# MattAgostini/ECE1782-Smith-Waterman-CUDA

Hardware: AMD Instinct MI355X
Metric: GCUPS (DP cell updates/s) query-vs-SwissProt, 1/2/4/8 MI355X; bit-exact scores (higher is better)
Workload: dtype fp16

## Files before the change

ece1782-smith-waterman-cuda_amd/csrc/sw_capi.cpp:

```cpp
#include <algorithm>
#include <cmath>
#include <atomic>
#include <cstdio>
#include <cstdlib>
#include <cstring>
#include <memory>
#include <new>
#include <numeric>
#include <string>
#include <thread>
#include <unordered_map>
#include <vector>

#include "sw_host.h"
#include "sw_plan.h"

using swk::DevPtr;
using swk::Event;
using swk::HostPtr;
using swk::Stream;

namespace {

thread_local std::string g_err;
// ... 1085 lines not shown
    }
    if ((p.multi_inter || p.multi_intra) && (rc = ensure_bnd(db, p.affine, p.intra_x2))) return rc;
    if (p.intra_x2 && !db->lay.d_lrescue.get()) {
        HIPCHECK(swk::dev_alloc(db->lay.d_lrescue, 2 * lstride * sizeof(int32_t)));
        HIPCHECK(hipMemsetAsync(db->lay.d_lrescue.get(), 0xff, 2 * lstride * sizeof(int32_t), h->stream.get()));
        db->lay.device_bytes += 2 * lstride * sizeof(int32_t);
    }
    if (db->list_epoch != g_fault_epoch.load()) {
        if ((rc = join_tails(h))) return rc;
        hipStream_t const s = h->stream.get();
        if (int32_t* l = db->lay.d_rescue.get()) HIPCHECK(hipMemsetAsync(l, 0xff, 2 * rstride * sizeof(int32_t), s));
        if (int32_t* l = db->lay.d_lrescue.get()) HIPCHECK(hipMemsetAsync(l, 0xff, 2 * lstride * sizeof(int32_t), s));
        db->list_epoch = g_fault_epoch.load();
    }
    c.par = h->parity;
    h->parity ^= 1;
    if (h->tail_pending[c.par]) {
        HIPCHECK(hipStreamWaitEvent(h->stream.get(), h->tail_done[c.par].get(), 0));
        h->tail_pending[c.par] = false;
    }
    if (p.drain && (rc = join_tails(h))) return rc;
    if (db->lay.d_rescue.get()) {
        c.listA = db->lay.d_rescue.get() + c.par * rstride;
        c.listB = c.listA + db->nblocks + 1;
        c.maxA = c.listA + 2 * (db->nblocks + 1);
        c.headA = c.maxA + 2;
        if (p.lpt && h->opts.lpt_persist != 0) c.lpt_next = c.maxA + 1;
    }
    if (db->lay.d_lrescue.get()) {
        c.list1 = db->lay.d_lrescue.get() + c.par * lstride;
        c.list2 = c.list1 + db->nlong + 1;
        c.head1 = c.list2 + db->nlong + 1;
    }
    c.deferred = !p.drain && defer && (!(p.multi_inter || p.multi_intra) || ensure_rbnd(db, p.affine, p.intra_x2));
    return SW_OK;
}

int scan_profiles(Scan& c, const QuerySrc& src, const int8_t* mat) {
    const swplan::ScanPlan& p = c.plan;
    const bool d = p.drain;
    int32_t* const cA = (p.rescue && c.db->nblocks) ? c.listA : nullptr;
    int32_t* const c1 = p.intra_x2 ? c.list1 : nullptr;
    int32_t* const reset[10] = {cA, (cA && p.f16) ? c.listB : nullptr, (cA && p.f16) ? c.maxA : nullptr, c1,
                                c1 ? c.list2 : nullptr, d ? c.headA : nullptr, d ? c.headA + 1 : nullptr,
                                d ? c.head1 : nullptr, d ? c.head1 + 1 : nullptr, c.lpt_next};
    const int rc = build_profiles(c.h, src, mat, c.sc.go, p.affine,
                                  std::max({p.qpad_inter, p.qpad_rescue, p.qpad_coop, p.qpad_list, p.qpad_intra2}),
                                  p.shape.x2s || p.intra_x2, p.ri, p.qpad_intra, reset, &c.P);
    c.h->evpool[c.h->nscans - 1].merged = p.lpt;
    return rc;
}

int inter_args(Scan& c) {
    sw_db* db = c.db;
    const swplan::ScanPlan& p = c.plan;
    const int go = c.sc.go, ge = c.sc.ge;
    swk::InterArgs& a = c.a;
    a.residues = db->lay.d_res.get();
    a.blk_off = db->lay.d_blk_off.get();
    a.blk_groups = db->lay.d_blk_groups.get();
    a.blk_cols = db->lay.d_blk_cols.get();
    a.lane_ids = db->lay.d_lane_ids.get();
    a.nblocks = static_cast<int32_t>(db->nblocks);
    a.prof = c.P.dev + (p.shape.x2s ? c.P.off16 : c.P.off8);
    a.prof_stride = c.P.stride;
    a.qpad = p.qpad_inter;
    a.gap_open = go;
    a.gap_extend = ge;
    a.bnd_h = db->lay.d_bnd_h.get();
    a.bnd_f = db->lay.d_bnd_f.get();
    a.scores = c.scores;
    if (c.h->opts.trace_file[0]) {
        if (!db->lay.h_trace.get()) {
            db->lay.trace_entries = static_cast<size_t>(2 * db->nblocks + db->nlong + 8);
            HIPCHECK(swk::host_alloc(db->lay.h_trace, 32 * db->lay.trace_entries, hipHostMallocMapped));
            std::memset(db->lay.h_trace.get(), 0, 32 * db->lay.trace_entries);
        }
        HIPCHECK(hipHostGetDevicePointer(reinterpret_cast<void**>(&a.trace), db->lay.h_trace.get(), 0));
    }
    if (p.rescue) {
        a.rescue_count = c.listA;
        a.rescue_list = c.listA + 1;
        if (p.f16) a.rescue_max = c.maxA;
        const int zero = -kF16Span + 2 * ge;
        a.sat_limit = kF16Span - zero - 2 * std::max(c.sc.max_s, 1) - 26 * ge;
        for (int j = 0; j < 32; ++j) a.f16_step[j] = f16_pair(j * ge + zero);
        a.f16_gog = f16_pair(go - ge);
        a.f16_zero = f16_pair(zero);
        a.f16_diff[0] = f16_pair(4 * ge);
        a.f16_diff[1] = f16_pair(8 * ge);
        a.f16_diff[2] = f16_pair(16 * ge);
    }
    a.re_last = p.re_last;
    if (p.lpt) {
        a.blk_first = p.npair;
        a.blk_quad = p.nquad;
        a.blk_tri = p.ntri ? 1 : 0;
        a.blk_tail = static_cast<int32_t>(db->nblocks) - p.ntail;
    } else if (p.npair) {
        a.blk_base = p.nr;
        a.blk_first = std::max(p.npair, p.nr);
    } else {
        a.blk_first = p.ncoop;
    }
    return SW_OK;
}

void intra_args(Scan& c) {
    const sw_db* db = c.db;
    swk::IntraArgs& ia = c.ia;
    ia.residues = db->lay.d_lres.get();
    ia.subj_off = db->lay.d_loff.get();
    ia.subj_len = db->lay.d_llen.get();
    ia.subj_id = db->lay.d_lid.get();
    ia.nsubj = static_cast<int32_t>(db->nlong);
    ia.prof = c.P.dev + c.P.intra_off;
    ia.qpad = c.plan.qpad_intra;
    ia.gap_open = c.sc.go;
    ia.gap_extend = c.sc.ge;
    ia.bnd_h = db->lay.d_lbnd_h.get();
    ia.bnd_f = db->lay.d_lbnd_f.get();
    ia.scores = c.scores;
}

void intra_x2_args(Scan& c) {
    const swplan::ScanPlan& p = c.plan;
    const int go = c.sc.go, ge = c.sc.ge;
    swk::IntraArgs& x = c.x;
    x = c.ia;
    x.prof = c.P.dev + c.P.off16;
    x.prof_stride = c.P.stride;
    x.bias = p.affine ? 0 : go;
    x.qpad = p.qpad_intra2;
    const int zero = -kF16Span + 2 * ge;
    x.sat_limit = kF16Span - zero - 2 * std::max(c.sc.max_s, 1) - swk::intra_bias_rows(p.ri2) * ge;
    for (int j = 0; j < swk::kIntraSteps; ++j) x.f16_step[j] = f16_pair(j * ge + zero);
    x.f16_zero = f16_pair(zero);
    x.f16_gog = f16_pair(go - ge);
    int32_t* const flagged = p.intra_i16_first ? c.list2 : c.list1;
    x.rescue_count = flagged;
    x.rescue_list = flagged + 1;
}

int scan_args(Scan& c) {
    if (c.db->nlong) {
        intra_args(c);
        if (c.plan.intra_x2) intra_x2_args(c);
    }
    return c.db->nblocks ? inter_args(c) : SW_OK;
}

struct RescueStages {
    swk::InterArgs a16, a32;
    swk::IntraArgs i16, i32;
};
RescueStages rescue_stages(const Scan& c, const swk::IntraArgs& x, const BndRows& r, bool in_launch) {
    const swplan::ScanPlan& p = c.plan;
    auto items = [](int32_t* list) { return list ? list + 1 : nullptr; };
    int32_t* const l32 = p.f16 ? c.listB : c.listA;
    RescueStages s{c.a, c.a, x, c.ia};
    s.a16.bnd_h = s.a32.bnd_h = r.h;
    s.a16.bnd_f = s.a32.bnd_f = r.f;
    s.a16.qpad = p.qpad_list;
    s.a16.re_last = p.affine ? 32 : 48;
    s.a32.re_last = swplan::rescue_rows(p.affine);
    s.a16.rescue_list = items(c.listB);
    s.a16.rescue_count = c.listB;
    s.a16.rescue_max = nullptr;
    s.a32.prof = c.P.dev + c.P.off8;
    s.a32.qpad = p.qpad_rescue;
    s.a32.rescue_list = nullptr;
    s.a32.rescue_count = nullptr;
    s.i16.bnd_h = s.i32.bnd_h = r.lh;
    s.i16.bnd_f = s.i32.bnd_f = r.lf;
// ... 1158 lines not shown
```

ece1782-smith-waterman-cuda_amd/csrc/sw_inter_x2.hip:

```cpp
#include <algorithm>

#include "sw_int32.h"
#include "sw_intra_x2.h"
#include "sw_kernels.h"

namespace swk {

typedef short s2 __attribute__((ext_vector_type(2)));
typedef unsigned short u2 __attribute__((ext_vector_type(2)));

__device__ __forceinline__ s2 as_s2(uint32_t x) { return __builtin_bit_cast(s2, x); }
__device__ __forceinline__ uint32_t as_u32(s2 x) { return __builtin_bit_cast(uint32_t, x); }
__device__ __forceinline__ s2 max2(s2 a, s2 b) { return __builtin_elementwise_max(a, b); }
__device__ __forceinline__ s2 usub2(s2 a, u2 g) {
    return __builtin_bit_cast(s2, __builtin_elementwise_sub_sat(__builtin_bit_cast(u2, a), g));
}

__host__ __device__ constexpr int x2_row_dwords(int R) { return (R / 4) % 2 == 1 ? R : R + 4; }

constexpr int kImgCodes = kPadCode + 1;

template <int R>
struct __attribute__((aligned(16))) X2Lds {
    static constexpr int kImg = kImgCodes * x2_row_dwords(R);
// ... 12 lines not shown
        default: return static_cast<uint32_t>(q.w);
    }
}

template <int SG>
__device__ __forceinline__ void load_codes(uint32_t (&w)[SG / 4], const uint8_t* p, bool valid) {
    if (valid) {
        if constexpr (SG == 16) {
            const int4 v = *reinterpret_cast<const int4*>(p);
            w[0] = v.x; w[1] = v.y; w[2] = v.z; w[3] = v.w;
        } else if constexpr (SG == 8) {
            const int2 v = *reinterpret_cast<const int2*>(p);
            w[0] = v.x; w[1] = v.y;
        } else {
            w[0] = *reinterpret_cast<const uint32_t*>(p);
        }
    } else {
#pragma unroll
        for (int q = 0; q < SG / 4; ++q) w[q] = 0x19191919u;
    }
}

__device__ __forceinline__ uint32_t code_of(const uint32_t* w, int jj) { return (w[jj >> 2] >> (8 * (jj & 3))) & 0xffu; }

template <uint32_t RB>
__device__ __forceinline__ uint32_t code_row(const uint32_t* w, int jj, uint32_t base) {
    static_assert(RB < 256, "row stride must fit a byte");
    return __builtin_amdgcn_udot4(w[jj >> 2], RB << (8 * (jj & 3)), base, false);
}

template <int SG>
__device__ __forceinline__ void load_pairs(uint32_t (&v)[SG], const int32_t* p) {
#pragma unroll
    for (int q = 0; q < SG / 4; ++q) {
        const int4 t = *reinterpret_cast<const int4*>(p + 4 * q);
        v[4 * q] = t.x; v[4 * q + 1] = t.y; v[4 * q + 2] = t.z; v[4 * q + 3] = t.w;
    }
}

template <int SG>
__device__ __forceinline__ void store_pairs(int32_t* p, const uint32_t (&v)[SG]) {
#pragma unroll
    for (int q = 0; q < SG / 4; ++q)
        *reinterpret_cast<int4*>(p + 4 * q) = make_int4(v[4 * q], v[4 * q + 1], v[4 * q + 2], v[4 * q + 3]);
}

__device__ __forceinline__ uint32_t lo_lo(uint32_t a, uint32_t b) { return __builtin_amdgcn_perm(b, a, 0x05040100u); }
__device__ __forceinline__ uint32_t hi_lo(uint32_t a, uint32_t b) { return __builtin_amdgcn_perm(b, a, 0x05040302u); }
__device__ __forceinline__ uint32_t hi_hi(uint32_t a, uint32_t b) { return __builtin_amdgcn_perm(b, a, 0x07060302u); }

template <int SG, bool AFFINE>
__device__ __forceinline__ void load_bnd(uint32_t (&v)[SG], const uint32_t* bnd, uint64_t i) {
    if constexpr (AFFINE) {
        load_pairs<SG>(v, reinterpret_cast<const int32_t*>(bnd) + i);
    } else {
        const uint16_t* p = reinterpret_cast<const uint16_t*>(bnd) + i;
        uint32_t w[SG / 2];
        if constexpr (SG == 8) {
            const int4 t = *reinterpret_cast<const int4*>(p);
            w[0] = t.x; w[1] = t.y; w[2] = t.z; w[3] = t.w;
        } else {
            static_assert(SG == 4, "sub-group width");
            const int2 t = *reinterpret_cast<const int2*>(p);
            w[0] = t.x; w[1] = t.y;
        }
#pragma unroll
        for (int q = 0; q < SG; ++q) v[q] = w[q / 2];
    }
}
template <int SG, bool AFFINE>
__device__ __forceinline__ void store_bnd(uint32_t* bnd, uint64_t i, const uint32_t (&hb)[SG]) {
    if constexpr (AFFINE) {
        store_pairs<SG>(reinterpret_cast<int32_t*>(bnd) + i, hb);
    } else {
        uint16_t* p = reinterpret_cast<uint16_t*>(bnd) + i;
        uint32_t w[SG / 2];
#pragma unroll
        for (int q = 0; q < SG / 2; ++q) w[q] = lo_lo(hb[2 * q], hb[2 * q + 1]);
        if constexpr (SG == 8) *reinterpret_cast<int4*>(p) = make_int4(w[0], w[1], w[2], w[3]);
        else *reinterpret_cast<int2*>(p) = make_int2(w[0], w[1]);
    }
}

__device__ __forceinline__ uint32_t to_f16_bits(uint32_t v16) {
    return static_cast<uint32_t>(__builtin_bit_cast(uint16_t, static_cast<_Float16>(static_cast<int16_t>(v16))));
}

template <int R, bool F16>
__device__ __forceinline__ void stage_x2s(X2Lds<R>& L, const int16_t* __restrict__ prof, int stride, int s0,
                                          int lane, int bias, int bias0, int img, int hi0 = R) {
    constexpr int RD = x2_row_dwords(R);
    constexpr int PER = kImgCodes * (R / 8);
    constexpr uint32_t one = F16 ? 0x3c00u : 1u;
    const int n = img < 0 ? 2 * PER : PER;
    for (int t = lane; t < n; t += kLanes) {
        const int im = img < 0 ? t / PER : img;
        const int u = img < 0 ? t % PER : t;
        const int c = u / (R / 8);
        const int k = u % (R / 8);
        const int16_t* src = prof + static_cast<size_t>(c) * stride + s0 + im * hi0 + 8 * k;
        int4 v;
        if (im && (hi0 & 7)) {
            const int2 v0 = *reinterpret_cast<const int2*>(src), v1 = *reinterpret_cast<const int2*>(src + 4);
            v = make_int4(v0.x, v0.y, v1.x, v1.y);
        } else {
            v = *reinterpret_cast<const int4*>(src);
        }
        const uint32_t w[4] = {static_cast<uint32_t>(v.x), static_cast<uint32_t>(v.y), static_cast<uint32_t>(v.z),
                               static_cast<uint32_t>(v.w)};
        uint32_t o[8];
#pragma unroll
        for (int e = 0; e < 4; ++e) {
            const int s0v = static_cast<int16_t>(w[e] & 0xffffu), s1v = static_cast<int16_t>(w[e] >> 16);
            const int b0 = (F16 && k % 2 == 0 && e == 0) ? bias0 : 0;
            uint32_t a0 = static_cast<uint32_t>(s0v) & 0xffffu, a1 = static_cast<uint32_t>(s1v) & 0xffffu;
            if constexpr (F16) {
                a0 = to_f16_bits(static_cast<uint32_t>(s0v + bias + b0));
                a1 = to_f16_bits(static_cast<uint32_t>(s1v + bias));
            }
            o[2 * e] = im ? (a0 << 16) | one : a0 | (one << 16);
            o[2 * e + 1] = im ? (a1 << 16) | one : a1 | (one << 16);
        }
        int4* d = reinterpret_cast<int4*>((im ? L.hi : L.lo) + c * RD + 8 * k);
        d[0] = make_int4(o[0], o[1], o[2], o[3]);
        d[1] = make_int4(o[4], o[5], o[6], o[7]);
    }
}


typedef int v4i __attribute__((ext_vector_type(4)));
typedef __attribute__((address_space(3))) const v4i lds_int4;

__device__ __forceinline__ uint32_t lds_addr(const void* p) {
    return static_cast<uint32_t>(reinterpret_cast<uintptr_t>(p));
}

template <int N>
__device__ __forceinline__ void read_x2a(int4 (&pl)[N], int4 (&ph)[N], uint32_t& aa, uint32_t& ab, int k,
                                         uint32_t dep) {
    asm volatile("" : "+v"(aa), "+v"(ab) : "v"(dep));
    lds_int4* a = reinterpret_cast<lds_int4*>(static_cast<uintptr_t>(aa)) + N * k;
    lds_int4* b = reinterpret_cast<lds_int4*>(static_cast<uintptr_t>(ab)) + N * k;
#pragma unroll
    for (int q = 0; q < N; ++q) {
        pl[q] = __builtin_bit_cast(int4, a[q]);
        ph[q] = __builtin_bit_cast(int4, b[q]);
    }
}

typedef _Float16 h2 __attribute__((ext_vector_type(2)));

template <bool F16>
struct PkCell;

template <>
struct PkCell<false> {
    using V = s2;
    static __device__ __forceinline__ V from(uint32_t x) { return as_s2(x); }
    static __device__ __forceinline__ uint32_t bits(V x) { return as_u32(x); }
};

template <>
struct PkCell<true> {
    using V = h2;
    static __device__ __forceinline__ V from(uint32_t x) { return __builtin_bit_cast(h2, x); }
    static __device__ __forceinline__ uint32_t bits(V x) { return __builtin_bit_cast(uint32_t, x); }
};

__device__ __forceinline__ h2 max3h(h2 a, h2 b, h2 c) {
    return __builtin_elementwise_maximum(__builtin_elementwise_maximum(a, b), c);
}

template <int R, int SG, bool AFFINE, bool F16, int CR = 16, bool SHORT = true>
__device__ __forceinline__ bool x2s_block(const InterArgs& a, int blk, X2Lds<R>& L, int lane);

template <int R, int SG, bool AFFINE, bool F16, bool LIST, int CR = 16>
__global__ __launch_bounds__(256, 2) void sw_inter_x2s(InterArgs a) {
    static_assert(R % CR == 0 && SG % 4 == 0, "shape");
    __shared__ __attribute__((aligned(16))) X2Lds<R> lds[kWavesPerWG];
    const int wave = __builtin_amdgcn_readfirstlane(threadIdx.x >> 6);
    const int lane = threadIdx.x & 63;
    X2Lds<R>& L = lds[wave];
    if constexpr (LIST) {
        const int n = __builtin_amdgcn_readfirstlane(*a.blk_count);
        for (int i = blockIdx.x * kWavesPerWG + wave; i < n; i += gridDim.x * kWavesPerWG)
            x2s_block<R, SG, AFFINE, F16, CR, false>(a, list_take(a.blk_list, i), L, lane);
        return;
    }
    const int blk = a.blk_first + blockIdx.x * kWavesPerWG + wave;
    if (blk >= a.nblocks) return;
    x2s_block<R, SG, AFFINE, F16, CR>(a, blk, L, lane);
}

constexpr int kRowGroup = 16;
constexpr int kAcc = kRowGroup + 8 - 1;
template <bool F16>
struct Best {
    typename PkCell<F16>::V v;
    __device__ __forceinline__ void init(const InterArgs&) { v = PkCell<F16>::from(0u); }
    __device__ __forceinline__ typename PkCell<F16>::V value(const InterArgs&) const { return v; }
};
template <>
struct Best<true> {
    h2 acc[kAcc];
    __device__ __forceinline__ void init(const InterArgs& a) {
#pragma unroll
        for (int k = 0; k < kAcc; ++k) acc[k] = __builtin_bit_cast(h2, a.f16_zero);
    }
    __device__ __forceinline__ void pin() {
        static_assert(kAcc == 23, "pin list");
        asm volatile("" : "+v"(acc[0]), "+v"(acc[1]), "+v"(acc[2]), "+v"(acc[3]), "+v"(acc[4]), "+v"(acc[5]),
                     "+v"(acc[6]), "+v"(acc[7]));
        asm volatile("" : "+v"(acc[8]), "+v"(acc[9]), "+v"(acc[10]), "+v"(acc[11]), "+v"(acc[12]), "+v"(acc[13]),
                     "+v"(acc[14]), "+v"(acc[15]));
        asm volatile("" : "+v"(acc[16]), "+v"(acc[17]), "+v"(acc[18]), "+v"(acc[19]), "+v"(acc[20]),
                     "+v"(acc[21]), "+v"(acc[22]));
    }
    __device__ __forceinline__ h2 value(const InterArgs& a) const {
        const h2 z = __builtin_bit_cast(h2, a.f16_step[0]);
        h2 b = acc[0];
#pragma unroll
        for (int k = 1; k < kAcc; ++k)
            b = __builtin_elementwise_maximum(b, acc[k] - (__builtin_bit_cast(h2, a.f16_step[k]) - z));
        return b;
    }
};

__device__ __forceinline__ uint64_t trace_now() {
#ifdef SW_TRACE_BLOCKS
    return __builtin_amdgcn_s_memrealtime();
#else
    return 0;
#endif
}
__device__ __forceinline__ void trace_block(const InterArgs& a, int blk, uint64_t t0, int lane, uint32_t kind) {
#ifdef SW_TRACE_BLOCKS
    if (a.trace && lane == 0) {
        const uint64_t t1 = __builtin_amdgcn_s_memrealtime();
        const uint32_t hw = __builtin_amdgcn_s_getreg((4) | (0 << 6) | (31 << 11));
        const uint32_t xcc = __builtin_amdgcn_s_getreg((20) | (0 << 6) | (31 << 11));
        uint64_t* t = a.trace + 4 * static_cast<size_t>(blk);
        t[0] = t0;
        t[1] = t1;
        t[2] = hw;
        t[3] = xcc | (static_cast<uint64_t>(kind) << 32);
    }
#else
    (void)a; (void)blk; (void)t0; (void)lane; (void)kind;
#endif
}

template <bool F16>
__device__ __forceinline__ bool x2s_finish(const InterArgs& a, int blk, int lane, typename PkCell<F16>::V best) {
    int b;
    if constexpr (F16)
        b = static_cast<int>(static_cast<float>(__builtin_elementwise_maximum(best.x, best.y))) -
            static_cast<int>(static_cast<float>(__builtin_bit_cast(h2, a.f16_step[0]).x));
    else
        b = max(static_cast<int>(best.x), static_cast<int>(best.y));
    const int id = a.lane_ids[static_cast<size_t>(blk) * kLanes + lane];
    if (id >= 0) a.scores[id] = b;
    if (a.rescue_list) {
        const bool sat = F16 ? (b >= a.sat_limit) : (b >= kSat16 || b < 0);
        const uint64_t m = __builtin_amdgcn_ballot_w64(sat);
        if (m && lane == 0) {
            list_publish(a.rescue_list, a.rescue_count, blk);
            if (a.rescue_max) atomicMax(a.rescue_max, blk);
        }
        return m != 0;
    }
    return false;
}


constexpr int kRingSlots = 4;

template <int SG>
__device__ __forceinline__ void ring_store(int4* ring, int slot, int lane, const uint32_t (&v)[SG]) {
#pragma unroll
    for (int q = 0; q < SG / 4; ++q)
        ring[(slot * (SG / 4) + q) * kLanes + lane] = make_int4(v[4 * q], v[4 * q + 1], v[4 * q + 2], v[4 * q + 3]);
}

template <int SG>
__device__ __forceinline__ void ring_load(uint32_t (&v)[SG], const int4* ring, int slot, int lane) {
#pragma unroll
    for (int q = 0; q < SG / 4; ++q) {
        const int4 t = ring[(slot * (SG / 4) + q) * kLanes + lane];
        v[4 * q] = static_cast<uint32_t>(t.x);
        v[4 * q + 1] = static_cast<uint32_t>(t.y);
        v[4 * q + 2] = static_cast<uint32_t>(t.z);
        v[4 * q + 3] = static_cast<uint32_t>(t.w);
    }
}

template <bool AFFINE>
constexpr bool pair_flags() { return AFFINE; }
struct PairSync {
    int* prog;
    int me;
    int base;
    int pred;
    int pred_base;
    int succ;
    int S;
};
__device__ __forceinline__ void pair_wait(const int* prog, int wave, int need) {
    while (__hip_atomic_load(prog + wave, __ATOMIC_ACQUIRE, __HIP_MEMORY_SCOPE_WORKGROUP) < need)
        __builtin_amdgcn_s_sleep(1);
}

template <int R, int SG, bool AFFINE, bool F16, bool PAIR, int CR = 16, bool CHAIN = false, int RL = R>
__device__ __forceinline__ void x2s_pass(const InterArgs& a, X2Lds<R>& L, uint32_t ncols, uint64_t base, int lane,
                                         int s0, Best<F16>& best, const int4* ring_in, int4* ring_out,
                                         int* tick, const PairSync* ps = nullptr, int chain_passes = 1) {
    static_assert(!(CHAIN && PAIR), "chained passes: single-wave blocks only");
    constexpr int CQ = CR / 4;
    constexpr int NCH = R / CR;
    constexpr int STEPS = SG * NCH;
    using P = PkCell<F16>;
    using V = typename P::V;
    const int16_t* prof16 = reinterpret_cast<const int16_t*>(a.prof);
    const u2 go2 = {static_cast<unsigned short>(a.gap_open), static_cast<unsigned short>(a.gap_open)};
    const u2 ge2 = {static_cast<unsigned short>(a.gap_extend), static_cast<unsigned short>(a.gap_extend)};
    uint32_t* bnd = reinterpret_cast<uint32_t*>(a.bnd_h);
    static_assert(!F16 || (R % kRowGroup == 0 && SG <= 8), "fp16 row groups");
    h2 gog_h = {}, reb_h = {}, grp_h = {};
    if constexpr (F16) {
        gog_h = __builtin_bit_cast(h2, a.f16_gog);
        static_assert(SG == 4 || SG == 8, "rebase constants");
        reb_h = __builtin_bit_cast(h2, a.f16_diff[SG == 4 ? 0 : 1]);
        grp_h = __builtin_bit_cast(h2, a.f16_diff[2]);
    }
    const bool first = (s0 == 0);
    const bool last = (s0 + 2 * R >= a.qpad);
    const uint32_t npass = CHAIN ? static_cast<uint32_t>(chain_passes) : 1u;
    const bool chain_last = CHAIN && static_cast<int>(npass) * 2 * R >= a.qpad;
    const uint32_t total = npass * ncols;
    const int sbias = F16 ? (AFFINE ? 2 : 1) * a.gap_extend : 0;
    const int gbias0 = F16 ? -kRowGroup * a.gap_extend : 0;
    const uint32_t dtop0 = F16 ? a.f16_step[SG - 2 + kRowGroup] : 0u;
    constexpr bool kSh = RL < R;
    if constexpr (kSh) asm volatile("" : "+v"(lane));
    static_assert(!kSh || (RL == R - 4 && !CHAIN), "rows per strip: R, or R - 4 outside a chain");
    static_assert((R - 4 - 1) % kRowGroup == 11, "the short strip's bottom row: 4 ge under the last row's bias");
    h2 dsh_h = {};
    if constexpr (F16) dsh_h = __builtin_bit_cast(h2, a.f16_diff[0]);
    stage_x2s<R, F16>(L, prof16, a.prof_stride, s0, lane, sbias, gbias0, -1, RL);
    __builtin_amdgcn_fence(__ATOMIC_RELEASE, "workgroup");
    __builtin_amdgcn_wave_barrier();
    __builtin_amdgcn_fence(__ATOMIC_ACQUIRE, "workgroup");

    V H[R];
    V E[AFFINE ? R : 1];
#pragma unroll
    for (int r = 0; r < R; ++r) H[r] = P::from(F16 ? a.f16_step[r % kRowGroup + SG - 1] : 0u);
#pragma unroll
    for (int r = 0; r < (AFFINE ? R : 1); ++r) E[r] = P::from(F16 ? a.f16_zero : 0u);
    uint32_t dtop = dtop0;
    uint32_t dl_h[SG], dl_f[SG];
    uint32_t bin[SG], bin_n[SG];
    uint32_t bz[SG];
    uint32_t rc[SG / 4], rp[SG / 4], rn[SG / 4];
#pragma unroll
    for (int q = 0; q < SG; ++q) {
        bz[q] = !F16 ? 0u
                     : AFFINE ? lo_lo(a.f16_step[kRowGroup - 1 + q], a.f16_step[kRowGroup + q])
                              : lo_lo(a.f16_step[kRowGroup - 1 + q], a.f16_step[kRowGroup - 1 + q]);
        dl_h[q] = F16 ? a.f16_step[kRowGroup - 1 + q] : 0u;
        dl_f[q] = F16 ? a.f16_step[kRowGroup + q] : 0u;
        bin[q] = bz[q];
        bin_n[q] = 0;
    }
#pragma unroll
    for (int q = 0; q < SG / 4; ++q) rp[q] = 0x19191919u;
    load_codes<SG>(rc, a.residues + base, true);
    constexpr bool kPairFlags = pair_flags<AFFINE>();
    auto wait_in = [&](uint32_t x) {
        if constexpr (PAIR && kPairFlags)
            pair_wait(ps->prog, ps->pred, ps->pred_base + min(static_cast<int>(x) + 2, ps->S));
    };
    if (!first) {
        wait_in(0);
        if (PAIR && ring_in) ring_load<SG>(bin, ring_in, 0, lane);
        else load_bnd<SG, AFFINE>(bin, bnd, base);
    }
    int4 PL[2][CQ], PH[2][CQ];
    constexpr uint32_t RB = x2_row_dwords(R) * 4;
    const uint32_t blo = lds_addr(L.lo), bhi = lds_addr(L.hi);
    uint32_t aa = code_row<RB>(rc, 0, blo), ab = bhi + kPadCode * RB;
    read_x2a<CQ>(PL[0], PH[0], aa, ab, 0, 0);

    uint32_t lo_p = 0, lo_c = 0;
    bool t2 = false;
    for (uint32_t col0 = 0; col0 <= total; col0 += SG) {
        const bool has_next = col0 + SG <= total;
        const bool next_lo = col0 + SG < total;
        const uint32_t ncol = col0 + SG;
        const bool wrap = CHAIN && lo_c + SG == ncols;
        const uint32_t nreal = CHAIN ? (wrap ? 0u : lo_c + SG) : ncol;
        const bool next_first = CHAIN ? (lo_p == 0 && !wrap) : first;
        const uint64_t noff = (nreal >> 4) * kGroupBytes + (nreal & 15);
        const bool t1 = CHAIN && lo_c == 0 && lo_p > 0 && lo_p < npass;
        const bool next_t1 = CHAIN && wrap && next_lo;
        const bool next_t2 = t1;
        if (t1) {
            stage_x2s<R, F16>(L, prof16, a.prof_stride, static_cast<int>(lo_p) * 2 * R, lane, sbias, gbias0, 0);
#pragma unroll
            for (int r = 0; r < R; ++r) {
                H[r] = P::from(__builtin_amdgcn_perm(P::bits(H[r]), F16 ? a.f16_step[r % kRowGroup + SG - 1] : 0u,
                                                     0x07060100u));
                if constexpr (AFFINE) E[r] = P::from(__builtin_amdgcn_perm(P::bits(E[r]), F16 ? a.f16_zero : 0u, 0x07060100u));
            }
            dtop = __builtin_amdgcn_perm(dtop, dtop0, 0x07060100u);
        }
        if (t2) {
            stage_x2s<R, F16>(L, prof16, a.prof_stride, static_cast<int>(lo_p) * 2 * R, lane, sbias, gbias0, 1);
#pragma unroll
            for (int r = 0; r < R; ++r) {
                H[r] = P::from(__builtin_amdgcn_perm(F16 ? a.f16_step[r % kRowGroup + SG - 1] : 0u, P::bits(H[r]),
                                                     0x07060100u));
                if constexpr (AFFINE) E[r] = P::from(__builtin_amdgcn_perm(F16 ? a.f16_zero : 0u, P::bits(E[r]), 0x07060100u));
            }
            dtop = __builtin_amdgcn_perm(dtop0, dtop, 0x07060100u);
        }
        if (t1 || t2) {
            __builtin_amdgcn_fence(__ATOMIC_RELEASE, "workgroup");
            __builtin_amdgcn_wave_barrier();
            __builtin_amdgcn_fence(__ATOMIC_ACQUIRE, "workgroup");
            aa = code_row<RB>(rc, 0, blo);
            ab = code_row<RB>(rp, 0, bhi);
            read_x2a<CQ>(PL[0], PH[0], aa, ab, 0, 0);
        }
        if (next_t1) {
            __builtin_amdgcn_fence(__ATOMIC_RELEASE, "workgroup");
            __builtin_amdgcn_fence(__ATOMIC_ACQUIRE, "workgroup");
        }
        if (has_next) {
            load_codes<SG>(rn, a.residues + base + noff, next_lo);
            if (!next_first && next_lo) {
                wait_in(ncol / SG);
                if (PAIR && ring_in) ring_load<SG>(bin_n, ring_in, (ncol / SG) % kRingSlots, lane);
                else load_bnd<SG, AFFINE>(bin_n, bnd, base + noff);
            }
        }
        if constexpr (F16) {
#pragma unroll
            for (int r = 0; r < R; ++r) {
                if (r <= RL) H[r] = H[r] - reb_h;
                if constexpr (AFFINE)
                    if (r < RL) E[r] = E[r] - reb_h;
            }
            dtop = P::bits(P::from(dtop) - reb_h);
        }
        auto cell = [&](const int r, const int jj, V& up, V& diag, V& f, const V slo, const V shi) {
            if constexpr (F16 && !AFFINE) {
                const int rg = r % kRowGroup;
                if (rg == 0 && r > 0) up = up - grp_h;
                const h2 t = max3h(H[r], up, __builtin_elementwise_fma(slo, shi, diag));
                const h2 h = __builtin_elementwise_maximum(t, __builtin_bit_cast(h2, a.f16_step[rg + jj]));
                h2& acc = best.acc[rg + jj];
                if (jj & 1) {
                    if (rg + 1 < kRowGroup) acc = max3h(acc, h, H[r + 1]);
                    else acc = __builtin_elementwise_maximum(acc, h);
                } else if (rg == 0) {
                    acc = __builtin_elementwise_maximum(acc, h);
                }
                diag = H[r];
                H[r] = h;
                up = h;
            } else if constexpr (!AFFINE) {
                const s2 h = usub2(max2(max2(H[r], up), slo * shi + diag), go2);
                diag = H[r];
                H[r] = h;
                up = h;
                best.v = max2(best.v, h);
            } else if constexpr (!F16) {
                const s2 h = max2(max2(E[r], f), slo * shi + diag);
                const s2 n = usub2(h, go2);
                E[r] = max2(usub2(E[r], ge2), n);
                f = max2(usub2(f, ge2), n);
                diag = H[r];
                H[r] = h;
                up = h;
                best.v = max2(best.v, h);
            }
        };
        auto cell_d = [&](const int r, const int jj, V& up, V& diag, V& f, const V d) {
          if constexpr (F16 && AFFINE) {
            const int rg = r % kRowGroup;
            if (rg == 0 && r > 0) f = f - grp_h;
            const h2 h = max3h(E[r], f, d);
            const h2 m = h - gog_h;
            E[r] = __builtin_elementwise_maximum(E[r], m);
            f = max3h(f, m, __builtin_bit_cast(h2, a.f16_step[rg + jj + 1]));
            h2& acc = best.acc[rg + jj];
            if (jj & 1) {
                if (rg + 1 < kRowGroup) acc = max3h(acc, h, H[r + 1]);
                else acc = __builtin_elementwise_maximum(acc, h);
            } else if (rg == 0) {
                acc = __builtin_elementwise_maximum(acc, h);
            }
            diag = H[r];
            H[r] = h;
            up = h;
          }
        };
        auto col_done = [&](const V up, const V f, const int jj) {
            if constexpr (kSh && F16) {
                dl_h[jj] = P::bits(up + dsh_h);
                if constexpr (AFFINE) dl_f[jj] = P::bits(f + dsh_h);
            } else {
                dl_h[jj] = P::bits(up);
                if constexpr (AFFINE) dl_f[jj] = P::bits(f);
            }
        };
        auto col_start = [&](V& up, V& diag, V& f, const int jj) {
            const uint32_t u = (AFFINE || jj % 2 == 0) ? lo_lo(bin[jj], dl_h[jj]) : hi_lo(bin[jj], dl_h[jj]);
            up = P::from(u);
            if constexpr (F16 && !AFFINE) up = up - grp_h;
            diag = P::from(dtop);
            dtop = u;
            if constexpr (AFFINE) f = P::from(hi_lo(bin[jj], dl_f[jj]));
            if constexpr (F16) f = f - grp_h;
        };
        V up = P::from(0u), diag = P::from(0u), f = P::from(0u);
#pragma unroll
        for (int t = 0; t < STEPS; ++t) {
            const int jj = t / NCH;
            const int k = t % NCH;
            const uint32_t dep = P::bits(k == 0 ? H[R - 1] : H[CR * k - 1]);
            if (t + 1 < STEPS) {
                const int jn = (t + 1) / NCH, kn = (t + 1) % NCH;
                if (kn == 0) {
                    aa = code_row<RB>(rc, jn, blo);
                    ab = code_row<RB>(rp, jn, bhi);
                }
                read_x2a<CQ>(PL[(t + 1) & 1], PH[(t + 1) & 1], aa, ab, kn, dep);
            } else if (has_next && !next_t1 && !next_t2) {
                aa = code_row<RB>(rn, 0, blo);
                ab = code_row<RB>(rc, 0, bhi);
                read_x2a<CQ>(PL[(t + 1) & 1], PH[(t + 1) & 1], aa, ab, 0, dep);
            }
            if (k == 0) col_start(up, diag, f, jj);
            const int4(&pl)[CQ] = PL[t & 1];
            const int4(&ph)[CQ] = PH[t & 1];
            const int n = RL - CR * k < CR ? (RL - CR * k > 0 ? RL - CR * k : 0) : CR;
            if constexpr (F16 && AFFINE) {
                V dd[CR];
#pragma unroll
                for (int i = 0; i < CR; ++i)
                    if (i < n)
                        dd[i] = __builtin_elementwise_fma(P::from(word(pl, i)), P::from(word(ph, i)),
                                                          i == 0 ? diag : H[CR * k + i - 1]);
#pragma unroll
                for (int i = 0; i < CR; ++i)
                    if (i < n) asm volatile("" : "+v"(dd[i]));
#pragma unroll
                for (int i = 0; i < CR; ++i)
                    if (i < n) cell_d(CR * k + i, jj, up, diag, f, dd[i]);
            } else {
#pragma unroll
                for (int i = 0; i < CR; ++i)
                    if (i < n) cell(CR * k + i, jj, up, diag, f, P::from(word(pl, i)), P::from(word(ph, i)));
            }
            if (k == NCH - 1) col_done(up, f, jj);
            if constexpr (!F16) asm volatile("" : "+v"(best.v));
            else best.pin();
            __builtin_amdgcn_sched_barrier(0);
        }
        const bool high_last = CHAIN ? chain_last && (lo_c == 0 ? lo_p : lo_p + 1) >= npass : last;
        if (!high_last && col0 >= SG) {
            uint32_t hb[SG];
#pragma unroll
            for (int q = 0; q < SG; ++q) hb[q] = AFFINE ? hi_hi(dl_h[q], dl_f[q]) : hi_hi(dl_h[q], dl_h[q]);
            const uint32_t pc = CHAIN ? (lo_c == 0 ? ncols - SG : lo_c - SG) : col0 - SG;
            if (PAIR && ring_out) {
                if constexpr (kPairFlags) {
                    const int x = static_cast<int>(pc / SG);
                    pair_wait(ps->prog, ps->succ, x >= kRingSlots ? ps->base + x - kRingSlots + 1 : ps->base - 2);
                }
                ring_store<SG>(ring_out, (pc / SG) % kRingSlots, lane, hb);
            } else {
                const uint64_t poff = (pc >> 4) * kGroupBytes + (pc & 15);
                store_bnd<SG, AFFINE>(bnd, base + poff, hb);
            }
        }
        if (has_next) {
#pragma unroll
            for (int q = 0; q < SG / 4; ++q) {
                rp[q] = rc[q];
                rc[q] = rn[q];
            }
#pragma unroll
            for (int q = 0; q < SG; ++q) bin[q] = (next_first || !next_lo) ? bz[q] : bin_n[q];
        }
        if constexpr (PAIR && kPairFlags) {
            __builtin_amdgcn_fence(__ATOMIC_RELEASE, "workgroup");
            __hip_atomic_store(ps->prog + ps->me, ps->base + static_cast<int>(col0 / SG) + 1, __ATOMIC_RELAXED,
                               __HIP_MEMORY_SCOPE_WORKGROUP);
        } else if constexpr (PAIR) {
            __syncthreads();
            ++*tick;
        }
        if constexpr (CHAIN) {
            t2 = t1;
            lo_c = nreal;
            lo_p += wrap ? 1u : 0u;
        }
    }
}

__device__ __forceinline__ uint32_t block_cols(const InterArgs& a, int blk) {
    return a.blk_cols ? a.blk_cols[blk] : a.blk_groups[blk] * kGroupCols;
}

template <int R, int SG, bool AFFINE, bool F16, int CR, bool SHORT>
__device__ __forceinline__ bool x2s_block(const InterArgs& a, int blk, X2Lds<R>& L, int lane) {
    const uint32_t ncols = block_cols(a, blk);
    const uint64_t base = a.blk_off[blk] + static_cast<uint64_t>(lane) * kGroupCols;
    Best<F16> best;
    best.init(a);
    const uint64_t t0 = trace_now();
    const bool sh = SHORT && a.re_last == R - 4 && (ncols < 32 || ncols >= 64);
    const int full_end = a.qpad - (sh ? 2 * R : 0);
    const int chained = ncols >= 32 ? full_end / (2 * R) : 0;
    int s0 = 0;
    if (chained > 1) {
        x2s_pass<R, SG, AFFINE, F16, false, CR, true>(a, L, ncols, base, lane, 0, best, nullptr, nullptr, nullptr,
                                                      nullptr, chained);
        s0 = chained * 2 * R;
    }
    for (; s0 < full_end && ncols > 0; s0 += 2 * R)
        x2s_pass<R, SG, AFFINE, F16, false, CR>(a, L, ncols, base, lane, s0, best, nullptr, nullptr, nullptr);
    if constexpr (SHORT) {
        if (sh && ncols > 0)
            x2s_pass<R, SG, AFFINE, F16, false, CR, false, R - 4>(a, L, ncols, base, lane, full_end, best, nullptr,
// ... 364 lines not shown
```

ece1782-smith-waterman-cuda_amd/csrc/sw_plan.cpp:

```cpp
#include "sw_plan.h"

#include <algorithm>
#include <cmath>
#include <cstdio>
#include <utility>
#include <vector>

namespace swplan {

namespace {
int32_t round_up(int64_t v, int64_t m) { return static_cast<int32_t>((v + m - 1) / m * m); }
}


constexpr int64_t kSmallDbSubjects = 64 * 1000;

constexpr double kFillSubjects = 570000.0;

int32_t default_long_threshold(const PlanDb& db) {
    if (db.n == 0) return 1536;
    const double mean = static_cast<double>(db.residues) / static_cast<double>(db.n);
    if (db.n < kSmallDbSubjects && mean >= 256) return 64;
    const double fill = db.n < kSmallDbSubjects ? 1.0 : std::min(1.0, static_cast<double>(db.n) / kFillSubjects);
    const double t = 5.7 * mean * std::pow(fill, 0.4);
// ... 183 lines not shown
            v = InterShape{r, g};
    }
    return v;
}

std::string inter_kernel_name(const swk::InterShape& v, bool affine) {
    char b[96];
    if (v.x2s)
        std::snprintf(b, sizeof b, "sw_inter_x2s<%d,%d,%s%s>", v.R / 2, v.SG, affine ? "affine" : "linear",
                      v.f16 ? ",fp16" : "");
    else
        std::snprintf(b, sizeof b, "sw_inter<%d,%d,%s>", v.R, v.SG, affine ? "affine" : "linear");
    return b;
}

int rescue_rows(bool affine) { return affine ? 32 : 64; }

int intra_rows_for(int qlen, int longest) {
    int best_ri = 16;
    double best_cost = 1e300;
    for (int ri = 2; ri <= 16; ri += 2) {
        const int chunk = swk::kLanes * ri;
        const int nch = (qlen + chunk - 1) / chunk;
        const double cost = static_cast<double>(nch) * (longest + swk::kLanes - 1) * (ri * 3.7 + 8.0);
        if (cost < best_cost) { best_cost = cost; best_ri = ri; }
    }
    return best_ri;
}

int intra_x2_rows_for(int qlen, int longest, int wide, int forced) {
    if (forced > 0) {
        const int ri = forced;
        if (ri == 4 || ri == 6 || ri == 8 || ri == 10 || ri == 12 || ri == 16) return ri;
        if (ri == swk::kIntraX2MaxRI && wide >= 1) return ri;
    }
    int best_ri = 16;
    double best_cost = 1e300;
    for (int ri : {4, 6, 8, 10, 12, 16, swk::kIntraX2MaxRI}) {
        if (ri == swk::kIntraX2MaxRI && wide < 2) continue;
        const int chunk = swk::kLanes * ri;
        const int nch = (qlen + chunk - 1) / chunk;
        const double cost = static_cast<double>(nch) * (longest + swk::kLanes - 1) * (ri * 28.8 + 80.0);
        if (cost < best_cost) {
            best_cost = cost;
            best_ri = ri;
        }
    }
    return best_ri;
}

bool lpt_supported(int ri) { return ri == 4 || ri == 6 || ri == 8; }

int32_t short_rows(int32_t qlen, int pass_rows) {
    const int32_t left = qlen - (round_up(qlen, pass_rows) / pass_rows - 1) * pass_rows;
    return (left + 1) / 2 <= pass_rows / 2 - 4 ? pass_rows / 2 - 4 : pass_rows / 2;
}

PlanScoring plan_scoring(const int8_t* m, int go, int ge) {
    PlanScoring s;
    s.go = go;
    s.ge = ge;
    for (int k = 0; k < 625; ++k) {
        s.max_s = std::max<int>(s.max_s, m[k]);
        if (m[k] + go > 127) s.biased_fits = false;
    }
    return s;
}

PlanScoring plan_scoring_max(int max_entry, int go, int ge) {
    PlanScoring s;
    s.go = go;
    s.ge = ge;
    s.max_s = std::max(0, max_entry);
    s.biased_fits = max_entry + go <= 127;
    return s;
}

PlanScoring plan_scoring_pssm(const int8_t* rows, int32_t qlen, int go, int ge) {
    int mx = -128;
    for (int64_t k = 0; k < static_cast<int64_t>(qlen) * 25; ++k) mx = std::max<int>(mx, rows[k]);
    return plan_scoring_max(mx, go, ge);
}

ScanPlan scan_plan(const PlanDb& db, int32_t qlen, const PlanScoring& s, bool intra_i16_first, int32_t i16_span) {
    const sw_opts& O = *db.opts;
    const int max_s = s.max_s, go = s.go, ge = s.ge;
    ScanPlan p;
    p.affine = go != ge || !s.biased_fits;
    const bool affine = p.affine;
    const bool f16_fits = 2 * max_s + 27 * ge + go < 1024;
    p.x2_ok = !f16_fits                                                   ? 0
              : (static_cast<int64_t>(qlen) + 2) * (max_s + go) < 32767 ? 2
              : (max_s + go < 1000 && ge < 1000)                       ? 1
                                                                       : 0;
    p.shape = inter_shape(affine, p.x2_ok, O);
    const int R = p.shape.R;
    p.rescue = swk::inter_needs_rescue(p.shape, p.x2_ok);
    p.f16 = p.shape.f16;
    p.qpad_rescue = p.rescue ? round_up(qlen, rescue_rows(affine)) : 0;
    const int list_rows = affine ? 64 : 96;
    p.qpad_list = p.f16 ? round_up(qlen, list_rows) : 0;

    p.intra_x2 = db.nlong && p.x2_ok >= 1 && O.intra_x2 != 0;
    p.intra_i16_first = intra_i16_first && p.intra_x2;
    const bool ri2_wide =
        db.nblocks == 0 && 2 * max_s + (swk::intra_bias_rows(swk::kIntraX2MaxRI) + 1) * ge + go < 1024;
    const int ri2_model =
        p.intra_x2 ? intra_x2_rows_for(qlen, db.long_max, ri2_wide ? (affine ? 2 : 1) : 0, O.intra_x2_rows) : 0;
    const int ri2_lpt = (affine && ri2_model > 8 && db.nblocks && O.intra_x2_rows < 0) ? 8 : ri2_model;

    p.npair = (db.nblocks && swk::inter_has_pair(p.shape) && round_up(qlen, R) > R) ? pair_blocks(db) : 0;
    p.ncoop = (!p.npair && db.nblocks) ? coop_blocks(db, swk::inter_coop_divisor(p.shape)) : 0;
    p.qpad_coop = p.ncoop ? round_up(qlen, swk::kCoopRows) : 0;
    p.nr = (p.f16 && p.rescue && p.npair && !p.ncoop) ? i16_span : 0;

    const bool lpt_want = O.lpt >= 0 ? O.lpt == 1 : true;
    p.lpt = lpt_want && db.nlong && db.nblocks && p.intra_x2 && !p.intra_i16_first && p.f16 && p.rescue &&
            p.npair && !p.ncoop && i16_span == 0 && lpt_supported(ri2_lpt);
    p.lpt_rows = (p.lpt && !affine && O.lpt_rows != 64 && round_up(qlen, 96) > 96) ? 96 : 64;
    p.qpad_inter = round_up(qlen, p.lpt_rows == 96 ? 96 : R);
    p.re_last = p.shape.x2s ? short_rows(qlen, p.lpt_rows == 96 ? 96 : R) : 0;
    if (p.lpt) {
        const int passes = p.qpad_inter / p.lpt_rows;
        p.ntri = affine ? lpt_tri_blocks(db, p.npair, passes) : 0;
        p.nquad = p.ntri ? p.ntri : lpt_quad_blocks(db, p.npair);
        p.ntail = lpt_tail_blocks(db, p.npair, passes);
    }

    p.ri = db.nlong ? intra_rows_for(qlen, db.long_max) : 0;
    p.qpad_intra = p.ri ? round_up(qlen, static_cast<int64_t>(swk::kLanes) * p.ri) : 0;
    p.ri2 = p.lpt ? ri2_lpt : ri2_model;
    p.qpad_intra2 = p.ri2 ? round_up(qlen, static_cast<int64_t>(swk::kLanes) * p.ri2) : 0;
    p.multi_inter = p.qpad_inter > R || p.qpad_rescue > rescue_rows(affine) || p.qpad_coop > swk::kCoopRows ||
                    p.qpad_list > list_rows;
    p.multi_intra = (p.ri && p.qpad_intra > swk::kLanes * p.ri) || (p.ri2 && p.qpad_intra2 > swk::kLanes * p.ri2);

    if (db.nblocks) {
        p.kernel = inter_kernel_name(p.shape, affine);
        if (p.npair) p.kernel.replace(0, sizeof("sw_inter_x2s") - 1, "sw_inter_x2p");
        if (p.lpt_rows == 96) p.kernel.replace(p.kernel.find("<32,"), 4, "<48,");
        if (p.nr) p.kernel += "+int16[0," + std::to_string(p.nr) + ")";
        if (p.ntail) p.kernel += "+tail" + std::to_string(p.ntail);
        if (p.ntri) p.kernel += "+tri" + std::to_string(p.ntri);
        if (p.lpt) p.kernel += "+lpt";
    }
    p.intra_kernel = !db.nlong   ? "none"
                     : p.intra_x2 ? "sw_intra_x2<" + std::to_string(p.ri2) + (p.intra_i16_first ? ",int16>" : ">")
                                  : "sw_intra<" + std::to_string(p.ri) + (affine ? ",affine>" : ",linear>");
    return p;
}

void ScanPlan::set_drain(bool got_rows) {
    if (!lpt || !got_rows || drain) return;
    drain = true;
    ri = ri2;
    qpad_intra = qpad_intra2;
    multi_intra = qpad_intra > swk::kLanes * ri;
    kernel += "+drain";
}

}
```

ece1782-smith-waterman-cuda_amd/csrc/sw_plan.h:

```cpp
#pragma once

#include <cstdint>
#include <string>
#include <vector>

#include "sw_amd.h"
#include "sw_kernels.h"

namespace swplan {

struct PlanDb {
    int64_t n = 0;
    int64_t residues = 0;
    int64_t nblocks = 0;
    int64_t nlong = 0;
    int32_t long_threshold = 0;
    int32_t long_max = 0;
    const uint32_t* blk_groups = nullptr;
    const int32_t* llen = nullptr;
    const sw_opts* opts = nullptr;
    int cus = 0;
};

int32_t default_long_threshold(const PlanDb& db);
int32_t coop_blocks(const PlanDb& db, int divisor);
int pair_group(const PlanDb& db);
int32_t pair_blocks(const PlanDb& db);
int32_t lpt_quad_blocks(const PlanDb& db, int32_t npair);
int32_t lpt_tri_blocks(const PlanDb& db, int32_t npair, int passes);
int32_t lpt_tail_blocks(const PlanDb& db, int32_t npair, int passes);
double intra_step_us(int ri);
double single_ticks(int64_t ncols, int passes);
double group_ticks_host(int64_t ncols, int passes, int G);

swk::InterShape inter_shape(bool affine, int x2_ok, const sw_opts& o);
std::string inter_kernel_name(const swk::InterShape& v, bool affine);
int rescue_rows(bool affine);
int intra_rows_for(int qlen, int longest);
int intra_x2_rows_for(int qlen, int longest, int wide, int forced);
bool lpt_supported(int ri);
int32_t short_rows(int32_t qlen, int pass_rows);

struct PlanScoring {
    int max_s = 0;
    int go = 0, ge = 0;
    bool biased_fits = true;
};
PlanScoring plan_scoring(const int8_t* matrix625, int go, int ge);
PlanScoring plan_scoring_pssm(const int8_t* rows, int32_t qlen, int go, int ge);
PlanScoring plan_scoring_max(int max_entry, int go, int ge);

struct ScanPlan {
    bool affine = false;
    int x2_ok = 0;
    swk::InterShape shape{};
    bool rescue = false;
    bool f16 = false;
    bool intra_x2 = false;
    bool intra_i16_first = false;
    int ri = 0;
    int ri2 = 0;
    int32_t qpad_inter = 0, qpad_intra = 0, qpad_intra2 = 0, qpad_rescue = 0, qpad_list = 0, qpad_coop = 0;
    int32_t npair = 0;
    int32_t ncoop = 0;
    int32_t nr = 0;
    bool lpt = false;
    bool drain = false;
    int lpt_rows = 64;
    int32_t re_last = 0;
    int32_t ntri = 0, nquad = 0, ntail = 0;
    bool multi_inter = false, multi_intra = false;
    std::string kernel, intra_kernel;

    void set_drain(bool got_rows);
};

ScanPlan scan_plan(const PlanDb& db, int32_t qlen, const PlanScoring& s, bool intra_i16_first, int32_t i16_span);

struct LptPlan {
    std::vector<int32_t> order;
    std::vector<float> cost;
    int32_t npipe = 0;
    int32_t pipe_tail = 0;
};
LptPlan lpt_plan(const PlanDb& db, int32_t qpad, int rows, int32_t qpad_intra, int ri, int32_t npair, int32_t nquad,
                 int32_t ntail, bool affine, bool tri);

}
```

Baseline: 11320.

## Replace fp16 arithmetic with integer ops on biased fp16 bit patterns

Switches the f16 inter-sequence kernel from fp16 arithmetic to integer add/subtract on the raw 16-bit patterns, offset by a bias of 0x2000 so every live value stays in the normal positive fp16 range. In that range the bit patterns are monotonic and evenly spaced, so fp16 max still orders them correctly while additions become plain 32-bit integer adds. The score profile is staged as biased integers instead of converted fp16 with a multiplier of 1, and the FMA becomes two integer adds. This trades packed fp16 FMA/sub for 32-bit integer adds, but a carry from the low half into the high half would corrupt the packed pair, and the headroom for saturation is recomputed through a new cell_range helper.

```diff
diff --git a/ece1782-smith-waterman-cuda_amd/csrc/sw_capi.cpp b/ece1782-smith-waterman-cuda_amd/csrc/sw_capi.cpp
--- a/ece1782-smith-waterman-cuda_amd/csrc/sw_capi.cpp
+++ b/ece1782-smith-waterman-cuda_amd/csrc/sw_capi.cpp
@@ -1191,14 +1191,12 @@
         a.rescue_count = c.listA;
         a.rescue_list = c.listA + 1;
         if (p.f16) a.rescue_max = c.maxA;
-        const int zero = -kF16Span + 2 * ge;
-        a.sat_limit = kF16Span - zero - 2 * std::max(c.sc.max_s, 1) - 26 * ge;
-        for (int j = 0; j < 32; ++j) a.f16_step[j] = f16_pair(j * ge + zero);
-        a.f16_gog = f16_pair(go - ge);
-        a.f16_zero = f16_pair(zero);
-        a.f16_diff[0] = f16_pair(4 * ge);
-        a.f16_diff[1] = f16_pair(8 * ge);
-        a.f16_diff[2] = f16_pair(16 * ge);
+        const swplan::CellRange cr = swplan::cell_range(-128, c.sc.max_s, go, ge);
+        a.sat_limit = cr.sat_limit;
+        std::copy(std::begin(cr.step), std::end(cr.step), a.f16_step);
+        a.f16_gog = cr.gog;
+        a.f16_zero = cr.step[0];
+        std::copy(std::begin(cr.diff), std::end(cr.diff), a.f16_diff);
     }
     a.re_last = p.re_last;
     if (p.lpt) {
diff --git a/ece1782-smith-waterman-cuda_amd/csrc/sw_inter_x2.hip b/ece1782-smith-waterman-cuda_amd/csrc/sw_inter_x2.hip
--- a/ece1782-smith-waterman-cuda_amd/csrc/sw_inter_x2.hip
+++ b/ece1782-smith-waterman-cuda_amd/csrc/sw_inter_x2.hip
@@ -118,16 +118,13 @@
     }
 }
 
-__device__ __forceinline__ uint32_t to_f16_bits(uint32_t v16) {
-    return static_cast<uint32_t>(__builtin_bit_cast(uint16_t, static_cast<_Float16>(static_cast<int16_t>(v16))));
-}
 
 template <int R, bool F16>
 __device__ __forceinline__ void stage_x2s(X2Lds<R>& L, const int16_t* __restrict__ prof, int stride, int s0,
                                           int lane, int bias, int bias0, int img, int hi0 = R) {
     constexpr int RD = x2_row_dwords(R);
     constexpr int PER = kImgCodes * (R / 8);
-    constexpr uint32_t one = F16 ? 0x3c00u : 1u;
+    constexpr uint32_t one = 1u;
     const int n = img < 0 ? 2 * PER : PER;
     for (int t = lane; t < n; t += kLanes) {
         const int im = img < 0 ? t / PER : img;
@@ -149,13 +146,15 @@
         for (int e = 0; e < 4; ++e) {
             const int s0v = static_cast<int16_t>(w[e] & 0xffffu), s1v = static_cast<int16_t>(w[e] >> 16);
             const int b0 = (F16 && k % 2 == 0 && e == 0) ? bias0 : 0;
-            uint32_t a0 = static_cast<uint32_t>(s0v) & 0xffffu, a1 = static_cast<uint32_t>(s1v) & 0xffffu;
+            const uint32_t a0 = static_cast<uint32_t>(s0v) & 0xffffu, a1 = static_cast<uint32_t>(s1v) & 0xffffu;
             if constexpr (F16) {
-                a0 = to_f16_bits(static_cast<uint32_t>(s0v + bias + b0));
-                a1 = to_f16_bits(static_cast<uint32_t>(s1v + bias));
-            }
-            o[2 * e] = im ? (a0 << 16) | one : a0 | (one << 16);
-            o[2 * e + 1] = im ? (a1 << 16) | one : a1 | (one << 16);
+                const uint32_t w0 = static_cast<uint32_t>(s0v + bias + b0), w1 = static_cast<uint32_t>(s1v + bias);
+                o[2 * e] = im ? w0 << 16 : w0;
+                o[2 * e + 1] = im ? w1 << 16 : w1;
+            } else {
+                o[2 * e] = im ? (a0 << 16) | one : a0 | (one << 16);
+                o[2 * e + 1] = im ? (a1 << 16) | one : a1 | (one << 16);
+            }
         }
         int4* d = reinterpret_cast<int4*>((im ? L.hi : L.lo) + c * RD + 8 * k);
         d[0] = make_int4(o[0], o[1], o[2], o[3]);
@@ -205,6 +204,12 @@
 
 __device__ __forceinline__ h2 max3h(h2 a, h2 b, h2 c) {
     return __builtin_elementwise_maximum(__builtin_elementwise_maximum(a, b), c);
+}
+__device__ __forceinline__ h2 iadd(h2 a, h2 b) {
+    return __builtin_bit_cast(h2, __builtin_bit_cast(uint32_t, a) + __builtin_bit_cast(uint32_t, b));
+}
+__device__ __forceinline__ h2 isub(h2 a, h2 b) {
+    return __builtin_bit_cast(h2, __builtin_bit_cast(uint32_t, a) - __builtin_bit_cast(uint32_t, b));
 }
 
 template <int R, int SG, bool AFFINE, bool F16, int CR = 16, bool SHORT = true>
@@ -253,11 +258,11 @@
                      "+v"(acc[21]), "+v"(acc[22]));
     }
     __device__ __forceinline__ h2 value(const InterArgs& a) const {
-        const h2 z = __builtin_bit_cast(h2, a.f16_step[0]);
         h2 b = acc[0];
 #pragma unroll
         for (int k = 1; k < kAcc; ++k)
-            b = __builtin_elementwise_maximum(b, acc[k] - (__builtin_bit_cast(h2, a.f16_step[k]) - z));
+            b = __builtin_elementwise_maximum(
+                b, __builtin_bit_cast(h2, __builtin_bit_cast(uint32_t, acc[k]) - (a.f16_step[k] - a.f16_step[0])));
         return b;
     }
 };
@@ -289,11 +294,12 @@
 template <bool F16>
 __device__ __forceinline__ bool x2s_finish(const InterArgs& a, int blk, int lane, typename PkCell<F16>::V best) {
     int b;
-    if constexpr (F16)
-        b = static_cast<int>(static_cast<float>(__builtin_elementwise_maximum(best.x, best.y))) -
-            static_cast<int>(static_cast<float>(__builtin_bit_cast(h2, a.f16_step[0]).x));
-    else
+    if constexpr (F16) {
+        const uint32_t u = PkCell<F16>::bits(best);
+        b = static_cast<int>(max(u & 0xffffu, u >> 16)) - static_cast<int>(a.f16_step[0] & 0xffffu);
+    } else {
         b = max(static_cast<int>(best.x), static_cast<int>(best.y));
+    }
     const int id = a.lane_ids[static_cast<size_t>(blk) * kLanes + lane];
     if (id >= 0) a.scores[id] = b;
     if (a.rescue_list) {
@@ -390,7 +396,7 @@
     V H[R];
     V E[AFFINE ? R : 1];
 #pragma unroll
-    for (int r = 0; r < R; ++r) H[r] = P::from(F16 ? a.f16_step[r % kRowGroup + SG - 1] : 0u);
+    for (int r = 0; r < R; ++r) H[r] = P::from(F16 && r < RL ? a.f16_step[r % kRowGroup + SG - 1] : 0u);
 #pragma unroll
     for (int r = 0; r < (AFFINE ? R : 1); ++r) E[r] = P::from(F16 ? a.f16_zero : 0u);
     uint32_t dtop = dtop0;
@@ -483,17 +489,17 @@
         if constexpr (F16) {
 #pragma unroll
             for (int r = 0; r < R; ++r) {
-                if (r <= RL) H[r] = H[r] - reb_h;
+                if (r < RL) H[r] = isub(H[r], reb_h);
                 if constexpr (AFFINE)
-                    if (r < RL) E[r] = E[r] - reb_h;
-            }
-            dtop = P::bits(P::from(dtop) - reb_h);
+                    if (r < RL) E[r] = isub(E[r], reb_h);
+            }
+            dtop -= P::bits(reb_h);
         }
         auto cell = [&](const int r, const int jj, V& up, V& diag, V& f, const V slo, const V shi) {
             if constexpr (F16 && !AFFINE) {
                 const int rg = r % kRowGroup;
-                if (rg == 0 && r > 0) up = up - grp_h;
-                const h2 t = max3h(H[r], up, __builtin_elementwise_fma(slo, shi, diag));
+                if (rg == 0 && r > 0) up = isub(up, grp_h);
+                const h2 t = max3h(H[r], up, iadd(iadd(slo, shi), diag));
                 const h2 h = __builtin_elementwise_maximum(t, __builtin_bit_cast(h2, a.f16_step[rg + jj]));
                 h2& acc = best.acc[rg + jj];
                 if (jj & 1) {
@@ -525,9 +531,9 @@
         auto cell_d = [&](const int r, const int jj, V& up, V& diag, V& f, const V d) {
           if constexpr (F16 && AFFINE) {
             const int rg = r % kRowGroup;
-            if (rg == 0 && r > 0) f = f - grp_h;
+            if (rg == 0 && r > 0) f = isub(f, grp_h);
             const h2 h = max3h(E[r], f, d);
-            const h2 m = h - gog_h;
+            const h2 m = isub(h, gog_h);
             E[r] = __builtin_elementwise_maximum(E[r], m);
             f = max3h(f, m, __builtin_bit_cast(h2, a.f16_step[rg + jj + 1]));
             h2& acc = best.acc[rg + jj];
@@ -544,8 +550,8 @@
         };
         auto col_done = [&](const V up, const V f, const int jj) {
             if constexpr (kSh && F16) {
-                dl_h[jj] = P::bits(up + dsh_h);
-                if constexpr (AFFINE) dl_f[jj] = P::bits(f + dsh_h);
+                dl_h[jj] = P::bits(iadd(up, dsh_h));
+                if constexpr (AFFINE) dl_f[jj] = P::bits(iadd(f, dsh_h));
             } else {
                 dl_h[jj] = P::bits(up);
                 if constexpr (AFFINE) dl_f[jj] = P::bits(f);
@@ -554,11 +560,11 @@
         auto col_start = [&](V& up, V& diag, V& f, const int jj) {
             const uint32_t u = (AFFINE || jj % 2 == 0) ? lo_lo(bin[jj], dl_h[jj]) : hi_lo(bin[jj], dl_h[jj]);
             up = P::from(u);
-            if constexpr (F16 && !AFFINE) up = up - grp_h;
+            if constexpr (F16 && !AFFINE) up = isub(up, grp_h);
             diag = P::from(dtop);
             dtop = u;
             if constexpr (AFFINE) f = P::from(hi_lo(bin[jj], dl_f[jj]));
-            if constexpr (F16) f = f - grp_h;
+            if constexpr (F16) f = isub(f, grp_h);
         };
         V up = P::from(0u), diag = P::from(0u), f = P::from(0u);
 #pragma unroll
@@ -587,8 +593,7 @@
 #pragma unroll
                 for (int i = 0; i < CR; ++i)
                     if (i < n)
-                        dd[i] = __builtin_elementwise_fma(P::from(word(pl, i)), P::from(word(ph, i)),
-                                                          i == 0 ? diag : H[CR * k + i - 1]);
+                        dd[i] = P::from(word(pl, i) + word(ph, i) + P::bits(i == 0 ? diag : H[CR * k + i - 1]));
 #pragma unroll
                 for (int i = 0; i < CR; ++i)
                     if (i < n) asm volatile("" : "+v"(dd[i]));
diff --git a/ece1782-smith-waterman-cuda_amd/csrc/sw_plan.cpp b/ece1782-smith-waterman-cuda_amd/csrc/sw_plan.cpp
--- a/ece1782-smith-waterman-cuda_amd/csrc/sw_plan.cpp
+++ b/ece1782-smith-waterman-cuda_amd/csrc/sw_plan.cpp
@@ -289,6 +289,23 @@
     return plan_scoring_max(mx, go, ge);
 }
 
+CellRange cell_range(int min_s, int max_s, int go, int ge) {
+    CellRange c;
+    c.z = 0x2000;
+    const int ms = std::max(max_s, 1), abs_s = std::max({ms, -min_s, 0});
+    auto pair = [](int v) { return static_cast<uint32_t>(v) * 0x00010001u; };
+    for (int j = 0; j < 32; ++j) c.step[j] = pair(j * ge + c.z);
+    c.gog = pair(go - ge);
+    c.diff[0] = pair(4 * ge);
+    c.diff[1] = pair(8 * ge);
+    c.diff[2] = pair(16 * ge);
+    c.sat_limit = 4096 - 28 * ge - 2 * ms;
+    c.lowest = c.z - go - 27 * ge - 2 * abs_s;
+    c.guard = c.z + c.sat_limit;
+    c.top = c.guard + 2 * ms + 26 * ge;
+    return c;
+}
+
 ScanPlan scan_plan(const PlanDb& db, int32_t qlen, const PlanScoring& s, bool intra_i16_first, int32_t i16_span) {
     const sw_opts& O = *db.opts;
     const int max_s = s.max_s, go = s.go, ge = s.ge;
diff --git a/ece1782-smith-waterman-cuda_amd/csrc/sw_plan.h b/ece1782-smith-waterman-cuda_amd/csrc/sw_plan.h
--- a/ece1782-smith-waterman-cuda_amd/csrc/sw_plan.h
+++ b/ece1782-smith-waterman-cuda_amd/csrc/sw_plan.h
@@ -75,6 +75,19 @@
     void set_drain(bool got_rows);
 };
 
+constexpr int kCellMin = 0x0400, kCellMax = 0x7BFF;
+struct CellRange {
+    int z = 0;
+    uint32_t step[32] = {};
+    uint32_t gog = 0;
+    uint32_t diff[3] = {};
+    int sat_limit = 0;
+    int lowest = 0;
+    int guard = 0;
+    int top = 0;
+};
+CellRange cell_range(int min_s, int max_s, int go, int ge);
+
 ScanPlan scan_plan(const PlanDb& db, int32_t qlen, const PlanScoring& s, bool intra_i16_first, int32_t i16_span);
 
 struct LptPlan {
```

Result: faster. 11590 (median of 6 runs) (+2.4%).
